# Nuttoty/Structured_Light_for_3D_Model_Replication

Hardware: AMD Instinct MI355X
Metric: decoded+triangulated px/s (higher is better)
Workload: dtype u8+f64

## Files before the change

### structured_light_for_3d_model_replication_amd/csrc/slgpu.hip

```cpp
#include <hip/hip_runtime.h>

#include <math.h>
#include <stdint.h>
#include <stdlib.h>
#include <string.h>

#include <stdio.h>

#include <algorithm>
#include <cmath>
#include <initializer_list>
#include <string>
#include <type_traits>
#include <thread>
#include <vector>

#include <dlfcn.h>
#include <errno.h>
#include <fcntl.h>
#include <sys/stat.h>
#include <unistd.h>

#include <chrono>
#include <condition_variable>
// ... 72 lines not shown
  int nc, nr, kc, kr;
  int mode;
  int Wp;
  const double4* planes;
  const float4* planes32;
  const double* xn;
  const double* yn;
  const float* xn32;
  const float* yn32;
  float fast_thr;
  int xy_safe;
  int xy_calc;
  double cx, cy, fx, fy;
  double rfx, rfy;
  const double* nc_rays;
  double o0, o1, o2;
  const double* poses;
  uint16_t* codes;
  int rec12;
  int rec_blk;
  uint8_t* ptnib;
  int32_t* col_out;
  int32_t* row_out;
  uint8_t* mask_out;
  void* xyz;
  uint8_t* bgr;
  int64_t out_cap;
  int64_t* view_offsets;
  ViewStats* stats;
  unsigned long long* masked;
  unsigned* hist;
  const int64_t* base_in;
  int* chunk_counts;
  int* block_sums;
  int bs_atomic;
  int decode_dyn;
  unsigned* super_base;
  unsigned* super_par;
  int sb_shift;
  int rerun;
  int cloud_gx;
  const uint8_t* pre_stack;
  int64_t pre_vs;
  unsigned* pre_hist;
  int pre_views;
  int pre_bpv;
};


__device__ __forceinline__ int64_t rec_slot(const Params& p, int view, int civ) {
  return (static_cast<int64_t>(civ >> 2) * p.n_views + view) * 4 + (civ & 3);
}

__device__ __forceinline__ uint4 ld16(const uint8_t* p, int n, bool vec) {
  if (vec) return *reinterpret_cast<const uint4*>(p);
  uint32_t w[4] = {0u, 0u, 0u, 0u};
#pragma unroll
  for (int i = 0; i < 16; ++i)
    if (i < n) w[i >> 2] |= static_cast<uint32_t>(p[i]) << (8 * (i & 3));
  return make_uint4(w[0], w[1], w[2], w[3]);
}

__device__ __forceinline__ uint32_t word(const uint4& q, int i) {
  return i == 0 ? q.x : i == 1 ? q.y : i == 2 ? q.z : q.w;
}

__device__ __forceinline__ uint32_t byte_of(const uint4& q, int i) {
  return (word(q, i >> 2) >> (8 * (i & 3))) & 0xffu;
}

__device__ __forceinline__ uint32_t gt_msb(uint32_t a, uint32_t b) {
  const uint32_t H = 0x80808080u;
  const uint32_t low = (a | H) - ((b & ~H) + 0x01010101u);
  return ((a & ~b) | (~(a ^ b) & low)) & H;
}

__device__ __forceinline__ uint32_t gt_bit7(uint32_t a, uint32_t b) {
  const uint32_t H = 0x80808080u;
  const uint32_t d = (b | H) - (a & ~H);
  return __builtin_amdgcn_bitop3_b32(a, b, d, 0x71);
}

__device__ __forceinline__ uint32_t gray_to_binary_bytes(uint32_t x, int bits) {
  if (bits > 1) x ^= (x >> 1) & 0x7f7f7f7fu;
// ... 255 lines not shown
}

template <int S>
__device__ __forceinline__ bool arrive_last(unsigned* ctr, unsigned id, unsigned readers) {
  const unsigned cls = id & (S - 1);
  const unsigned n_cls = (readers - cls + S - 1) / S;
  if (atomicAdd(ctr + 1 + cls, 1u) + 1u != n_cls) return false;
  return atomicAdd(ctr, 1u) + 1u == min(readers, static_cast<unsigned>(S));
}

__device__ __forceinline__ void hist_release(unsigned* h, int words, unsigned id, unsigned readers, int lane,
                                             uint32_t dep0, uint32_t dep1) {
  asm volatile("" ::"v"(dep0), "v"(dep1) : "memory");
  unsigned last = 0u;
  if (lane == 0) last = arrive_last<8>(h + kSlotArrive, id, readers) ? 1u : 0u;
  if (__shfl(static_cast<int>(last), 0, 64)) {
    uint4* h4 = reinterpret_cast<uint4*>(h);
    for (int i = lane; i < words / 4; i += 64) h4[i] = make_uint4(0u, 0u, 0u, 0u);
  }
}

__device__ __forceinline__ uint32_t mask4(uint32_t w, uint32_t b, uint32_t tw2, uint32_t tc2, uint32_t* bytes) {
  const uint32_t we = w & 0x00ff00ffu, wo = (w >> 8) & 0x00ff00ffu;
  const uint32_t be = b & 0x00ff00ffu, bo = (b >> 8) & 0x00ff00ffu;
  const uint32_t me = ((we | 0x80008000u) - tw2) & (((we + 0x00100010u) | 0x80008000u) - (be + tc2));
  const uint32_t mo = ((wo | 0x80008000u) - tw2) & (((wo + 0x00100010u) | 0x80008000u) - (bo + tc2));
  const uint32_t y = ((me >> 15) & 0x00010001u) | ((mo >> 7) & 0x01000100u);
  *bytes = y;
  return (y & 1u) | ((y >> 7) & 2u) | ((y >> 14) & 4u) | ((y >> 21) & 8u);
}

constexpr int kDecPl = 2048, kDecX = 4096, kDecY = 4096;
constexpr int kDecPlWords = kDecPl * 4;
constexpr int kBsSlots = 64;
constexpr int kSuperCap = 4096;
constexpr int kSuperWords = 2 * kSuperCap + 4;

__device__ __forceinline__ unsigned* super_produce(const Params& p) {
  const unsigned sel = p.super_par[0] & 1u;
  if (!p.rerun && blockIdx.x == 0 && blockIdx.y == 0) {
    unsigned* other = p.super_base + (sel ^ 1u) * kSuperCap;
    for (int i = threadIdx.x; i < kSuperCap; i += kThreads) other[i] = 0u;
    if (threadIdx.x == 0) p.super_par[1] = sel;
  }
  return p.super_base + sel * kSuperCap;
}
__device__ __forceinline__ const unsigned* super_consume(const Params& p, int bx) {
  const unsigned sel = p.super_par[1] & 1u;
  if (!p.rerun && bx == 0 && blockIdx.y == 0 && threadIdx.x == 0) p.super_par[0] = sel ^ 1u;
  return p.super_base + sel * kSuperCap;
}
constexpr int kDecodeLds = (kDecPlWords + kDecX) * 4;
static_assert(kDecodeLds >= 256 * kHistStride * 4, "the decode LDS holds the histogram replicas too");

constexpr int kDecodePerCu = 3;
template <int KC, int KR, int MODE, int VEC>
__global__ __launch_bounds__(kThreads, 3) void k_decode(Params p) {
  const int mode = MODE >= 0 ? MODE : p.mode;
  const int kc = KC >= 0 ? KC : p.kc;
  const int krr = (mode & M_ROWS) ? (KR >= 0 ? KR : p.kr) : 0;
  const int nc = p.nc, nr = p.nr;
  const bool vec = VEC > 0;
  const bool hist = (mode & M_HIST) && !(mode & M_DECIDE);

  __shared__ __attribute__((aligned(16))) unsigned s_lds[kDecodeLds / 4];
  __shared__ int s_max[kWaves];
  __shared__ int s_cnt[2][kWaves];
  __shared__ unsigned s_bsum[kBsSlots];
  __shared__ uint32_t s_thr[2];
  __shared__ unsigned s_mcount;
  __shared__ int s_next[2];
  __shared__ uint4 s_mapst[(MODE < 0 || (MODE & M_MAPS)) ? 64 * kWaves : 1];
  unsigned* s_hist = s_lds;
  float4* s_pl = reinterpret_cast<float4*>(s_lds);
  float* s_xn = reinterpret_cast<float*>(s_lds) + kDecPlWords;
  const bool decide = (mode & M_DECIDE) != 0;
  const int tid = threadIdx.x;
  const int lane = tid & 63;
  const int wid = __builtin_amdgcn_readfirstlane(tid >> 6);
  const int view = blockIdx.y;
  const int64_t HW = p.HW;
  const int gx = static_cast<int>(gridDim.x);
  if (decide) {
    if (tid < kBsSlots) s_bsum[tid] = 0u;
    if (tid == 0) s_mcount = 0u;
    if ((mode & M_HIST) && wid == 0) {
      const Thresholds t = view_thresholds(p, view, lane);
      if (lane == 0) {
        s_thr[0] = static_cast<uint32_t>(t.white + 1) * 0x00010001u;
        s_thr[1] = static_cast<uint32_t>(t.contrast + 17) * 0x00010001u;
        if (blockIdx.x == 0) {
          p.stats[view].thr_white = t.white;
          p.stats[view].thr_contrast = t.contrast;
          p.stats[view].noise_floor = t.noise_floor;
          p.stats[view].dynamic_range = t.dynamic_range;
        }
      }
    }
    if (mode & M_CODES) {
      const int wp_t = min(p.Wp, kDecPl), w_t = min(p.W, kDecX);
      typedef __attribute__((address_space(3))) void* lds_ptr_t;
      for (int i = wid; i * 64 < wp_t; i += kWaves)
        __builtin_amdgcn_global_load_lds(p.planes32 + min(i * 64 + lane, wp_t - 1), (lds_ptr_t)(s_pl + i * 64), 16, 0, 0);
      for (int i = wid; i * 256 < w_t; i += kWaves)
        __builtin_amdgcn_global_load_lds(p.xn32 + min(i * 256 + 4 * lane, w_t - 4), (lds_ptr_t)(s_xn + i * 256), 16, 0, 0);
    }
  }
  uint32_t tw2 = static_cast<uint32_t>(40 + 1) * 0x00010001u;
  uint32_t tc2 = static_cast<uint32_t>(10 + 17) * 0x00010001u;
  int it = 0;

  if (hist) {
    for (int i = tid; i < 256 * kHistStride; i += kThreads) s_hist[i] = 0u;
    __syncthreads();
  }

  const int ngroups = (p.cpv + kWaves - 1) / kWaves;
  int mx_acc = -1024;
  const bool dyn = p.decode_dyn && decide && (mode & M_CODES) && !p.bs_atomic;
  unsigned* const sup = (decide && (mode & M_CODES)) ? super_produce(p) : nullptr;
  unsigned* const dyn_ctr = sup + (kSuperCap - 1 - view);
  for (int cg = blockIdx.x; cg < ngroups;) {
  unsigned dyn_next = 0u;
  if (dyn && tid == 0) dyn_next = atomicAdd(dyn_ctr, 1u);
  const int civ = cg * kWaves + wid;
  const bool live = civ < p.cpv;
  const int64_t px0 = static_cast<int64_t>(civ) * kChunk + lane * kPx;
  const int n_px = live ? static_cast<int>(min<int64_t>(max<int64_t>(HW - px0, 0), kPx)) : 0;
  const int64_t pxl = n_px > 0 ? px0 : 0;
  const int64_t o = view * HW + px0;

  const float ys_early = (decide && (mode & M_CODES) && n_px > 0) ? p.yn32[row_of(p, static_cast<int>(px0))] : 0.0f;
  uint32_t col[kPx];
  uint32_t pt_rec = 0xffffu;
  uint4 wq = make_uint4(0u, 0u, 0u, 0u), bq = wq;
  uint32_t rA[4] = {0, 0, 0, 0}, rB[4] = {0, 0, 0, 0};
  const int rBn = krr > 8 ? krr - 8 : 0;
  const int rSh = nr - krr;
  if (mode & M_FROMMAPS) {
    const int64_t ol = view * HW + pxl;
    if (vec) {
      const int4* cm = reinterpret_cast<const int4*>(p.in_col + ol);
#pragma unroll
      for (int i = 0; i < 4; ++i) {
        const int4 v = cm[i];
        col[4 * i] = static_cast<uint32_t>(max(v.x, 0));
        col[4 * i + 1] = static_cast<uint32_t>(max(v.y, 0));
        col[4 * i + 2] = static_cast<uint32_t>(max(v.z, 0));
        col[4 * i + 3] = static_cast<uint32_t>(max(v.w, 0));
      }
    } else {
#pragma unroll
      for (int k = 0; k < kPx; ++k) col[k] = k < n_px ? static_cast<uint32_t>(max(p.in_col[ol + k], 0)) : 0u;
    }
  } else {
    const uint8_t* vbase = p.stack + view * p.stack_vs;
    const int voff = static_cast<int>(pxl);
    const __amdgpu_buffer_rsrc_t rs_view =
        __builtin_amdgcn_make_buffer_rsrc(const_cast<uint8_t*>(vbase), 0, p.view_bytes, 0x00020000);
// ... 180 lines not shown
      }
      const float ys = ys_early;
      uint32_t todo = ok;
      if (!(mode & M_NC)) {
#pragma unroll
        for (int k = 0; k < kPx; ++k) {
          const float a = fabsf(__builtin_fmaf(pf[k].x, xs[k], __builtin_fmaf(pf[k].y, ys, pf[k].z)));
          if (a > p.fast_thr) pt |= 1u << k;
        }
        pt &= ok;
        todo &= ~pt;
      }
#pragma unroll
      for (int k = 0; k < kPx; ++k) {
        if (!((todo >> k) & 1u)) continue;
        const int c = static_cast<int>(min(col[k], static_cast<uint32_t>(p.Wp - 1)));
        const int64_t q = px0 + k;
        float x, y, z, inv;
        if (mode & M_NC) {
          x = static_cast<float>(p.nc_rays[q]);
          y = static_cast<float>(p.nc_rays[HW + q]);
          z = static_cast<float>(p.nc_rays[2 * HW + q]);
          inv = 1.0f;
        } else {
          x = xs[k];
          y = ys;
          z = 1.0f;
          inv = __frsqrt_rn(x * x + y * y + 1.0f);
        }
        if (has_point(p, mode, pf[k], c, x, y, z, inv, u0 + k, v, q)) pt |= 1u << k;
      }
    }
    if (mode & M_CODES) {
      const int64_t gci = static_cast<int64_t>(view) * p.cpv + civ;
      pt_rec = pt;
      const int cnt = wave_sum_dpp(__popc(pt));
      if (lane == 0) {
        if (live) p.chunk_counts[gci] = cnt;
        const unsigned mine = live ? static_cast<unsigned>(cnt) : 0u;
        if (p.bs_atomic) {
          const unsigned old = atomicAdd(&s_bsum[it], (1u << 16) | mine);
          if ((old >> 16) == kWaves - 1) {
            const int64_t blk = static_cast<int64_t>(view) * ngroups + cg;
            const unsigned t = (old & 0xffffu) + mine;
            p.block_sums[blk] = static_cast<int>(t);
            if (t) atomicAdd(sup + (blk >> p.sb_shift), t);
          }
        } else {
          s_cnt[it & 1][wid] = static_cast<int>(mine);
        }
      }
    }
  }
  if (hist) {
    unsigned* hrow = s_hist + (lane & (kHistRep - 1));
    int mx = -1024;
#pragma unroll
    for (int k = 0; k < kPx; ++k) {
      if (k < n_px) {
        const int bk = static_cast<int>(byte_of(bq, k));
        atomicAdd(hrow + bk * kHistStride, 1u);
        mx = max(mx, static_cast<int>(byte_of(wq, k)) - bk);
      }
    }
    mx_acc = max(mx_acc, mx);
  }

  if (mode & M_CODES) {
    uint32_t rec[kPx / 2];
#pragma unroll
    for (int i = 0; i < kPx / 2; ++i)
      rec[i] = min(col[2 * i], static_cast<uint32_t>(p.Wp - 1)) |
               (min(col[2 * i + 1], static_cast<uint32_t>(p.Wp - 1)) << 16);
    if (decide) {
      const bool blk = !(mode & M_MAPS);
      if (n_px == kPx) {
        uint32_t rw[6];
        uint32_t* ro = blk ? rw : reinterpret_cast<uint32_t*>(reinterpret_cast<uint8_t*>(p.codes) + 3 * o / 2);
#pragma unroll
        for (int h = 0; h < 2; ++h) {
          const uint32_t* r = rec + 4 * h;
          auto cd = [&](int k, uint32_t c) { return ((pt_rec >> (8 * h + k)) & 1u) ? c : 0xfffu; };
          const uint32_t c0 = cd(0, r[0] & 0xffffu), c1 = cd(1, r[0] >> 16), c2 = cd(2, r[1] & 0xffffu);
          const uint32_t c3 = cd(3, r[1] >> 16), c4 = cd(4, r[2] & 0xffffu), c5 = cd(5, r[2] >> 16);
          const uint32_t c6 = cd(6, r[3] & 0xffffu), c7 = cd(7, r[3] >> 16);
          ro[3 * h] = c0 | (c1 << 12) | (c2 << 24);
          ro[3 * h + 1] = (c2 >> 8) | (c3 << 4) | (c4 << 16) | (c5 << 28);
          ro[3 * h + 2] = (c5 >> 4) | (c6 << 8) | (c7 << 20);
        }
        if (blk) {
          const __amdgpu_buffer_rsrc_t rs = __builtin_amdgcn_make_buffer_rsrc(
              reinterpret_cast<uint8_t*>(p.codes) + kRecSlot * rec_slot(p, view, civ), 0, kRecSlot, 0x00020000);
          __builtin_amdgcn_raw_buffer_store_b128(v4u{rw[0], rw[1], rw[2], rw[3]}, rs, 16 * lane, 0, kRecAux);
          __builtin_amdgcn_raw_buffer_store_b64(v2u{rw[4], rw[5]}, rs, 1024 + 8 * lane, 0, kRecAux);
        }
      }
    } else if (vec) {
      if (n_px == kPx) {
        uint4* ro = reinterpret_cast<uint4*>(p.codes + o);
        ro[0] = make_uint4(rec[0], rec[1], rec[2], rec[3]);
        ro[1] = make_uint4(rec[4], rec[5], rec[6], rec[7]);
      }
    } else {
#pragma unroll
      for (int k = 0; k < kPx; ++k)
        if (k < n_px) p.codes[o + k] = static_cast<uint16_t>(rec[k >> 1] >> (16 * (k & 1)));
    }
  }
  if (decide && (mode & M_CODES) && !p.bs_atomic) {
    if (dyn && tid == 0) s_next[it & 1] = static_cast<int>(dyn_next) + gx;
    __syncthreads();
    if (tid == 0) {
      int t = 0;
#pragma unroll
      for (int w = 0; w < kWaves; ++w) t += s_cnt[it & 1][w];
      const int64_t blk = static_cast<int64_t>(view) * ngroups + cg;
      p.block_sums[blk] = t;
      if (t) atomicAdd(sup + (blk >> p.sb_shift), static_cast<unsigned>(t));
    }
  }
  cg = dyn ? s_next[it & 1] : cg + gx;
  ++it;
  }

  if (decide && p.masked) {
    __syncthreads();
    if (tid == 0 && s_mcount) atomicAdd(p.masked + view, static_cast<unsigned long long>(s_mcount));
  }
  if (decide && (mode & M_HIST) && !p.rerun && wid == 0)
    hist_release(p.hist + static_cast<int64_t>(view) * kHistView, kHistView, blockIdx.x, gx, lane, tw2, tc2);

  if (hist) {
#pragma unroll
    for (int d = 32; d > 0; d >>= 1) mx_acc = max(mx_acc, __shfl_xor(mx_acc, d, 64));
    if (lane == 0) s_max[wid] = mx_acc;
    __syncthreads();
    unsigned* gh = p.hist + view * kSlot;
    unsigned cnt = 0u;
    const unsigned* row = s_hist + tid * kHistStride;
#pragma unroll
    for (int r = 0; r < kHistRep; ++r) cnt += row[r];
    if (cnt) atomicAdd(gh + tid, cnt);
    if (tid == 0) {
      int m = s_max[0];
#pragma unroll
      for (int w = 1; w < kWaves; ++w) m = max(m, s_max[w]);
      if (m > -1024) atomicMax(gh + 256, static_cast<unsigned>(m + 1024));
    }
  }
}

template <int VEC>
__device__ __forceinline__ int count_chunk(const Params& p, int64_t gc, int view, int civ, int lane, bool live,
                                           int* masked) {
// ... 185 lines not shown
          u -= W;
          ++v;
        }
        const int64_t q = static_cast<int64_t>(cpx) + 256 * s + 4 * lane + e;
        float x, y, z, inv;
        if (nc) {
          x = static_cast<float>(p.nc_rays[q]);
          y = static_cast<float>(p.nc_rays[p.HW + q]);
          z = static_cast<float>(p.nc_rays[2 * p.HW + q]);
          inv = 1.0f;
        } else {
          x = xs[e];
          y = vec ? ys : p.yn32[v];
          z = 1.0f;
          inv = __frsqrt_rn(x * x + y * y + 1.0f);
        }
        if (has_point(p, mode, pf[e], c, x, y, z, inv, u, v, q)) nib |= 1u << e;
      }
    }
    total += __popc(nib);
    nibs[s] = nib;
  }
#pragma unroll
  for (int s = 0; s < 4; ++s) p.ptnib[gc * kChunkNib + 64 * s + lane] = static_cast<uint8_t>(nibs[s]);
  if ((mode & M_MAPS) && vec) {
    uint8_t* mo_ = p.mask_out + static_cast<int64_t>(view) * HW;
#pragma unroll
    for (int s = 0; s < 4; ++s) {
      const int px = cpx + 256 * s + 4 * lane;
      if (px < HW) __builtin_nontemporal_store(mbytes[s], reinterpret_cast<uint32_t*>(mo_ + px));
    }
  }
  total = wave_sum(total);
  if (lane == 0) p.chunk_counts[gc] = total;
  return total;
}

template <int VEC>
__global__ __launch_bounds__(kThreads, 1) void k_count(Params p) {
  __shared__ int s_sum[kWaves];
  __shared__ int s_msum[kWaves];
  const int lane = threadIdx.x & 63;
  const int wid = __builtin_amdgcn_readfirstlane(threadIdx.x >> 6);
  const int view = blockIdx.y;
  const int civ = blockIdx.x * kWaves + wid;
  const int64_t gc = static_cast<int64_t>(view) * p.cpv + civ;
  int mc = 0;
  const int total = count_chunk<VEC>(p, gc, view, civ, lane, civ < p.cpv, &mc);
  if (p.masked) {
    mc = wave_sum(mc);
    if (lane == 0) s_msum[wid] = mc;
    __syncthreads();
    if (threadIdx.x == 0) {
      int t = 0;
#pragma unroll
      for (int w = 0; w < kWaves; ++w) t += s_msum[w];
      if (t) atomicAdd(p.masked + view, static_cast<unsigned long long>(t));
    }
  }
  if (!(p.mode & M_CODES)) return;
  unsigned* const sup = super_produce(p);
  if (lane == 0) s_sum[wid] = total;
  __syncthreads();
  if (threadIdx.x == 0) {
    int t = 0;
#pragma unroll
    for (int w = 0; w < kWaves; ++w) t += s_sum[w];
    const int64_t blk = static_cast<int64_t>(view) * gridDim.x + blockIdx.x;
    p.block_sums[blk] = t;
    if (t) atomicAdd(sup + (blk >> p.sb_shift), static_cast<unsigned>(t));
  }
}

constexpr int kPipe = 4;
constexpr int kBgrWords = 3 * kChunk / 4 + 4;

template <typename T>
__device__ __forceinline__ T* at_bytes(T* base, unsigned off) {
  using B = typename std::conditional<std::is_const<T>::value, const char, char>::type;
  return reinterpret_cast<T*>(reinterpret_cast<B*>(base) + off);
}

__device__ __forceinline__ uint32_t ent_code(uint32_t e) { return (e >> 10) & 0x7fffu; }
template <int VEC>
__device__ __forceinline__ void chunk_uv(int u_c, int v_c, uint32_t e, int W, int* u, int* v) {
  const int local = static_cast<int>(e & 1023u);
  int uu = u_c + local, vv = v_c;
  if (VEC > 0) {
    const int dr = static_cast<int>(e >> 25);
    uu -= dr * W;
    vv += dr;
  } else if (W >= kChunk) {
    const bool wrap = uu >= W;
    uu -= wrap ? W : 0;
    vv += wrap ? 1 : 0;
  } else {
    while (uu >= W) {
      uu -= W;
      ++vv;
    }
  }
  __builtin_assume(uu >= 0 && uu < (1 << 24));
// ... 423 lines not shown
      t4[3 * lane] = tq[0];
      t4[3 * lane + 1] = tq[1];
      t4[3 * lane + 2] = tq[2];
    } else {
      t4[lane] = tq[0];
    }
  }
  {
    int idx = incl - n_l;
#pragma unroll
    for (int k = 0; k < kPx; ++k) {
      const uint32_t code = (d[k >> 1] >> (16 * (k & 1))) & 0x7fffu;
      if ((ptbits >> k) & 1u) s_ent[idx] = static_cast<uint32_t>(lane * kPx + k) | (code << 10) | drow;
      idx += (ptbits >> k) & 1u;
    }
  }
  __builtin_amdgcn_wave_barrier();
  cloud_points<MODE, VEC, PIPE>(p, view, cpx, base, lane, total, s_ent, s_bgr);
}

constexpr int kPrefixBatch = 4;

__device__ __forceinline__ long long block_offset(const Params& p, const unsigned* sup, int64_t b, int tid, int lane,
                                                  int wid, long long* s_wred) {
  long long acc = 0;
  const int64_t sb = b >> p.sb_shift;
  for (int64_t t0 = 0; t0 < sb; t0 += kPrefixBatch * kThreads) {
    unsigned v[kPrefixBatch];
#pragma unroll
    for (int i = 0; i < kPrefixBatch; ++i) v[i] = sup[min<int64_t>(t0 + i * kThreads + tid, sb - 1)];
#pragma unroll
    for (int i = 0; i < kPrefixBatch; ++i) acc += (t0 + i * kThreads + tid < sb) ? v[i] : 0u;
  }
  for (int64_t t0 = sb << p.sb_shift; t0 < b; t0 += kPrefixBatch * kThreads) {
    int v[kPrefixBatch];
#pragma unroll
    for (int i = 0; i < kPrefixBatch; ++i) v[i] = p.block_sums[min<int64_t>(t0 + i * kThreads + tid, b - 1)];
#pragma unroll
    for (int i = 0; i < kPrefixBatch; ++i) acc += (t0 + i * kThreads + tid < b) ? v[i] : 0;
  }
  acc = wave_sum64(acc);
  if (lane == 0) s_wred[wid] = acc;
  __syncthreads();
  long long t = 0;
#pragma unroll
  for (int w = 0; w < kWaves; ++w) t += s_wred[w];
  return t;
}

constexpr int kExactPipe = 2;
constexpr int kVerifyPipe = 2;
static_assert(kWaves * kChunk >= 256 * kHistStride,
              "k_cloud's pre-stats workgroups keep their LDS histogram replicas in s_ent");
template <int MODE, int VEC, int PIPE>
__global__ __launch_bounds__(kThreads, 5) void k_cloud(Params p) {
  __shared__ uint32_t s_ent[kWaves][kChunk];
  __shared__ __attribute__((aligned(16))) uint32_t s_bgr[kWaves][kBgrWords];
  __shared__ long long s_wred[kWaves];
  const int tid = threadIdx.x;
  const int lane = tid & 63;
  const int wid = __builtin_amdgcn_readfirstlane(tid >> 6);
  const int view = blockIdx.y;
  const int npre = static_cast<int>(gridDim.x) - p.cloud_gx;
  if (static_cast<int>(blockIdx.x) < npre) {
    pre_stats_block(p, blockIdx.x, npre, &s_ent[0][0], reinterpret_cast<int*>(s_wred));
    return;
  }
  const int cx = static_cast<int>(blockIdx.x) - npre;
  const int civ = cx * kWaves + wid;
  const int64_t b = static_cast<int64_t>(view) * p.cloud_gx + cx;
  const int64_t gc = static_cast<int64_t>(view) * p.cpv + civ;
  const int before = (lane < wid && civ < p.cpv) ? p.chunk_counts[gc - wid + lane] : 0;
  long long base = block_offset(p, super_consume(p, cx), b, tid, lane, wid, s_wred);
  base += p.base_in ? *p.base_in : 0ll;
  base += wave_sum(before);
  base = uniform64(base);
  if (civ >= p.cpv) return;
  ChunkIn in;
  cloud_load<VEC>(p, gc, lane, &in);
  if (lane == 0 && view == p.n_views - 1 && civ == p.cpv - 1)
    p.view_offsets[p.n_views] = base + p.chunk_counts[gc];
  cloud_chunk<MODE, VEC, PIPE>(p, gc, base, lane, in, &s_ent[wid][0], &s_bgr[wid][0]);
}

}


struct sl_ctx {
  int device = 0;
  std::string err;
  bool has_calib = false;
  int H = 0, W = 0, Wp = 0;
  double Oc[3] = {0, 0, 0};
  double* d_planes = nullptr;
  double* d_xn = nullptr;
  double* d_yn = nullptr;
  float* d_f32 = nullptr;
  float fast_thr = 0.0f;
  bool xy_safe = false;
  bool xy_calc = false;
  bool xy_plain = false;
  bool planes_plain = false;
  double cam[4] = {0, 0, 1, 1};
  bool verify32 = true;
  double* d_nc = nullptr;
  ViewStats* d_stats = nullptr;
  int64_t cap_stats = 0;
  unsigned* d_hist[2] = {nullptr, nullptr};
  int64_t cap_hist = 0;
  int64_t hist_dirty[2] = {0, 0};
  unsigned long long cap_domain = 0;
  int* d_chunk_counts = nullptr;
  int64_t cap_cc = 0;
  int* d_block_sums = nullptr;
  int64_t cap_bs = 0;
  unsigned* d_super = nullptr;
  bool super_dirty = false;
  uint8_t* d_ptnib = nullptr;
  int64_t cap_ptnib = 0;
  uint16_t* d_codes = nullptr;
  int64_t cap_codes = 0;
  int last_views = 0;
  int decode_wgs = 0;
  int pre_wgs = 0;
  std::vector<hipEvent_t> prof_ev;
  std::vector<int> prof_groups;
  std::vector<char> prof_decide;
  int n_cu = 0;
  int prof_n = 0;
  void* comm = nullptr;
  int nranks = 0, rank = 0;
  int64_t* d_gcounts = nullptr;
  unsigned* d_ply_bsum = nullptr;
  int64_t cap_ply_bsum = 0;
  int64_t* d_ply_boff = nullptr;
  int64_t cap_ply_boff = 0;
  char* d_ply_text = nullptr;
  int64_t cap_ply_text = 0;
  char* h_ply_text = nullptr;
  int64_t cap_h_ply_text = 0;
  unsigned* d_plyr_state = nullptr;
  int64_t cap_plyr_state = 0;
  int64_t* d_plyr_tok = nullptr;
  int64_t cap_plyr_tok = 0;
  double* d_plyr_val = nullptr;
  int64_t cap_plyr_val = 0;
  int* d_plyr_cols = nullptr;
  int64_t cap_plyr_cols = 0;
// ... 89 lines not shown
      return fail((ctx), SL_EHIP, std::string(#expr) + ": " + hipGetErrorString(e_)); \
  } while (0)

int bit_count(int n) {
  int b = 0;
  while ((1ll << b) < n) ++b;
  return b;
}

int zero_async(sl_ctx* c, void* p, int64_t words, hipStream_t s);

template <typename T>
int grow(sl_ctx* c, T** ptr, int64_t* cap, int64_t need, hipStream_t s = nullptr, bool on_stream = false) {
  if (need <= *cap) return SL_OK;
  if (*ptr) HIP_TRY(c, hipFree(*ptr));
  *ptr = nullptr;
  const int64_t n = std::max<int64_t>(need, *cap * 2);
  const int64_t words = (static_cast<int64_t>(sizeof(T)) * n + 3) / 4;
  HIP_TRY(c, hipMalloc(reinterpret_cast<void**>(ptr), 4 * words));
  if (on_stream) {
    const int r = zero_async(c, *ptr, words, s);
    if (r) return r;
  } else {
    HIP_TRY(c, hipMemset(*ptr, 0, 4 * words));
    HIP_TRY(c, hipDeviceSynchronize());
  }
  *cap = n;
  return SL_OK;
}

int ensure_scratch(sl_ctx* c, int64_t views, int64_t px, bool codes, int64_t hist_views = 0,
                   bool* hist_fresh = nullptr, hipStream_t s = nullptr, bool on_stream = false) {
  const int64_t chunks = views * ((px + kChunk - 1) / kChunk);
  int r = grow(c, &c->d_chunk_counts, &c->cap_cc, chunks, s, on_stream);
  if (r) return r;
  r = grow(c, &c->d_block_sums, &c->cap_bs, views * (((px + kChunk - 1) / kChunk + kWaves - 1) / kWaves), s,
           on_stream);
  if (r) return r;
  r = grow(c, &c->d_ptnib, &c->cap_ptnib, chunks * kChunkNib, s, on_stream);
  if (r) return r;
  int64_t scap = c->d_super ? kSuperWords : 0;
  r = grow(c, &c->d_super, &scap, kSuperWords, s, on_stream);
  if (r) return r;
  const int64_t before = c->cap_hist, need = std::max(views, hist_views) * kHistView;
  for (int d = 0; d < 2; ++d) {
    int64_t cap = before;
    r = grow(c, &c->d_hist[d], &cap, need, s, on_stream);
    if (r) return r;
    if (d == 1) c->cap_hist = cap;
  }
  if (c->cap_hist != before) {
    c->hist_dirty[0] = c->hist_dirty[1] = 0;
    c->pre_armed = false;
    if (hist_fresh) *hist_fresh = true;
  }
  if (codes)
    return grow(c, &c->d_codes, &c->cap_codes,
                std::max<int64_t>(views * px, views * ((px + 4 * kChunk - 1) / (4 * kChunk)) * 4 * (kRecSlot / 2)) + 16,
                s, on_stream);
  return SL_OK;
}

using KernelFn = void (*)(Params);
constexpr int kProfGroups = 64;
constexpr int kProfEv = 4 * kProfGroups;

KernelFn pick_decode(int kc, int kr, int mode, bool vec) {
  if (vec && !(mode & (M_NC | M_FROMMAPS))) {
    constexpr int mrch = M_MAPS | M_ROWS | M_CODES | M_HIST, mrh = M_MAPS | M_ROWS | M_HIST,
                  ch = M_CODES | M_HIST, mrc = M_MAPS | M_ROWS | M_CODES, cc = M_CODES;
// ... 115 lines not shown
    pc.pre_views = pnv;
    pc.pre_bpv = static_cast<int>(bpv);
    const int64_t total = static_cast<int64_t>(pnv) * bpv;
    grid.x += static_cast<unsigned>((total + nv - 1) / nv);
    hist_dirty = static_cast<int64_t>(pnv) * kHistView;
  };
  bool next_pre = pre_use;
  int g = 0;
  for (int v0 = 0; v0 < p0.n_views; v0 += vpg, ++g) {
    hipEvent_t* gev = (ev && g < kProfGroups) ? ev + 4 * g : nullptr;
    if (gev) HIP_TRY(c, hipEventRecord(gev[0], s));
    const int nv = std::min(vpg, p0.n_views - v0);
    c->last_launch_px = static_cast<int64_t>(nv) * p0.HW;
    Params p = p0;
    p.n_views = nv;
    p.n_chunks = static_cast<int64_t>(nv) * cpv;
    if (p.stack) p.stack += v0 * p.stack_vs;
    if (p.tex) p.tex += v0 * p.tex_vs;
    if (p.in_col) p.in_col += v0 * p.HW;
    if (p.in_mask) p.in_mask += v0 * p.HW;
    if (p.col_out) p.col_out += v0 * p.HW;
    if (p.row_out) p.row_out += v0 * p.HW;
    if (p.mask_out) p.mask_out += v0 * p.HW;
    if (p.poses) p.poses += 16 * v0;
    if (p.masked) p.masked += v0;
    if (p.view_offsets) p.view_offsets += v0;
    p.base_in = (v0 > 0 && p.view_offsets) ? p.view_offsets : nullptr;
    p.stats = c->d_stats + v0;
    p.codes = c->d_codes;
    p.rec12 = (decide && cloud_mode >= 0) ? 1 : 0;
    p.rec_blk = (p.rec12 && !(decode_mode & M_MAPS)) ? 1 : 0;
    p.ptnib = c->d_ptnib;
    p.chunk_counts = c->d_chunk_counts;
    p.block_sums = c->d_block_sums;
    p.hist = hbuf;
    p.super_base = c->d_super;
    p.super_par = c->d_super + 2 * kSuperCap;
    const bool pre_g = next_pre;
    next_pre = false;
    const dim3 grid(static_cast<unsigned>((cpv + kWaves - 1) / kWaves), static_cast<unsigned>(nv));
    {
      const int64_t nb = static_cast<int64_t>(grid.x) * nv;
      int sh = 0;
      while ((int64_t{1} << (2 * sh)) < nb) ++sh;
      p.sb_shift = sh;
    }
    c->last.valid = true;
    dim3 dgrid = grid;
    if (c->decode_wgs > 0) dgrid.x = std::min(grid.x, static_cast<unsigned>(std::max(1, (c->decode_wgs + nv - 1) / nv)));
    c->last.grid[0] = dgrid;
    p.bs_atomic = decide && (grid.x + dgrid.x - 1) / dgrid.x <= static_cast<unsigned>(kBsSlots);
    p.decode_dyn = (!(decode_mode & M_MAPS) && decide && codes && dgrid.x < grid.x &&
                    ((static_cast<int64_t>(grid.x) * nv) >> p.sb_shift) + 1 + nv < kSuperCap) ? 1 : 0;
    if (p.decode_dyn) p.bs_atomic = 0;
    c->last.grid[1] = c->last.grid[2] = grid;
    c->last.s = s;
    c->last.fn[1] = c->last.fn[2] = nullptr;
    c->last.decide = decide;
    c->last.stats = false;
    if (decide) {
      if (adaptive) {
        const int64_t per_view = (p0.HW / 16 + kThreads - 1) / kThreads;
        const dim3 sg(static_cast<unsigned>(std::max<int64_t>(1, std::min<int64_t>(per_view, (2 * c->n_cu + nv - 1) / nv))),
                      static_cast<unsigned>(nv));
        p.mode = decode_mode;
        c->last.p[1] = p;
        c->last.grid[1] = sg;
        c->last.stats = true;
        if (!pre_g) {
          void* args[] = {&p};
          const void* kst = reinterpret_cast<const void*>(k_stats);
          c->last.fn[1] = kst;
          HIP_TRY(c, hipLaunchKernel(kst, sg, dim3(kThreads), args, 0, s));
        }
      }
      if (gev) HIP_TRY(c, hipEventRecord(gev[1], s));
    }
    if (codes) c->super_dirty = true;
    {
      p.mode = decode_mode;
      KernelFn fn = pick_decode(p.kc, (decode_mode & M_ROWS) ? p.kr : 0, decode_mode, vec);
      c->last.p[0] = p;
      c->last.p[0].masked = nullptr;
      c->last.fn[0] = reinterpret_cast<const void*>(fn);
      void* args[] = {&p};
      HIP_TRY(c, hipLaunchKernel(reinterpret_cast<const void*>(fn), dgrid, dim3(kThreads), args, 0, s));
      hist_dirty = (adaptive && !decide) ? static_cast<int64_t>(nv) * kSlot : 0;
// ... 442 lines not shown
    n_cu = 256;
  c->n_cu = n_cu;
  c->decode_wgs = kDecodePerCu * n_cu;
  c->pre_wgs = 2 * n_cu;
  if (const char* d = getenv("SLGPU_VERIFY32")) c->verify32 = atoi(d) != 0;
  if (hipEventCreateWithFlags(&c->done_ev, hipEventDisableTiming) != hipSuccess) {
    delete c;
    return SL_EHIP;
  }
  *out = c;
  return SL_OK;
}

void sl_ctx_destroy(sl_ctx* c) {
  if (!c) return;
  (void)hipSetDevice(c->device);
  if (c->comm) {
    if (Rccl* R = rccl()) (void)R->comm_destroy(static_cast<ncclComm_t>(c->comm));
  }
  if (c->d_gcounts) (void)hipFree(c->d_gcounts);
  for (void* ptr : {static_cast<void*>(c->d_ply_bsum), static_cast<void*>(c->d_ply_boff),
                    static_cast<void*>(c->d_ply_text), static_cast<void*>(c->d_plyr_state),
                    static_cast<void*>(c->d_plyr_tok), static_cast<void*>(c->d_plyr_val),
                    static_cast<void*>(c->d_plyr_cols)})
    if (ptr) (void)hipFree(ptr);
  if (c->h_ply_text) (void)hipHostFree(c->h_ply_text);
  slstream::ring_release(&c->file_ring);
  if (c->done_ev) (void)hipEventDestroy(c->done_ev);
  for (hipEvent_t e : c->prof_ev) (void)hipEventDestroy(e);
  for (void* ptr : {static_cast<void*>(c->d_planes), static_cast<void*>(c->d_xn), static_cast<void*>(c->d_yn),
                    static_cast<void*>(c->d_nc), static_cast<void*>(c->d_stats), static_cast<void*>(c->d_f32),
                    static_cast<void*>(c->d_codes), static_cast<void*>(c->d_hist[0]),
                    static_cast<void*>(c->d_hist[1]), static_cast<void*>(c->d_ptnib),
                    static_cast<void*>(c->d_block_sums), static_cast<void*>(c->d_chunk_counts),
                    static_cast<void*>(c->d_super)})
    if (ptr) (void)hipFree(ptr);
  delete c;
}

const char* sl_ctx_last_error(const sl_ctx* c) { return c ? c->err.c_str() : "null context"; }

int sl_ctx_reserve(sl_ctx* c, int64_t max_views, int64_t max_px) {
  if (!c || max_views < 1 || max_px < 1) return fail(c, SL_EINVAL, "sl_ctx_reserve: bad sizes");
  HIP_TRY(c, hipSetDevice(c->device));
  const int64_t vpg = std::max<int64_t>(1, kMaxChunks / ((max_px + kChunk - 1) / kChunk));
  int r = ensure_scratch(c, std::min(vpg, max_views), max_px, true, vpg);
  if (r) return r;
  return grow(c, &c->d_stats, &c->cap_stats, max_views);
}

int sl_set_calib(sl_ctx* c, int H, int W, const double* K, const double* Oc, const double* planes,
                 int Wp, const double* Nc) {
  if (!c) return SL_EINVAL;
  if (H < 1 || W < 1 || Wp < 1 || !K || !Oc || !planes)
    return fail(c, SL_EINVAL, "sl_set_calib: bad arguments");
  if (Wp > kMaxWp) return fail(c, SL_EINVAL, "sl_set_calib: at most 32768 projector columns");
  HIP_TRY(c, hipSetDevice(c->device));
  const double fx = K[0], fy = K[4], cx = K[2], cy = K[5];
  std::vector<double> xn(W), yn(H);
  for (int u = 0; u < W; ++u) xn[u] = (static_cast<double>(u) - cx) / fx;
  for (int v = 0; v < H; ++v) yn[v] = (static_cast<double>(v) - cy) / fy;
  bool use_nc = false;
  const int64_t HW = static_cast<int64_t>(H) * W;
  if (Nc) {
    for (int64_t q = 0; q < HW && !use_nc; ++q) {
      const double x = xn[q % W], y = yn[q / W];
      const double nrm = sqrt((x * x + y * y) + 1.0);
// ... 413 lines not shown
  hipError_t e = clear();
  if (e == hipSuccess && c->last.decide && c->last.stats) e = run(reinterpret_cast<const void*>(k_stats), 1);
  if (e == hipSuccess) e = run(c->last.fn[0], 0);
  if (e == hipSuccess && !c->last.decide && c->last.fn[1]) e = run(c->last.fn[1], 1);
  hipEvent_t ev[4] = {nullptr, nullptr, nullptr, nullptr};
  for (int k = 0; k < 4 && e == hipSuccess; ++k) e = hipEventCreate(&ev[k]);
  int r = e == hipSuccess ? SL_OK : fail(c, SL_EHIP, std::string("sl_time_kernels: ") + hipGetErrorString(e));
  const int order3[3] = {2, 1, 0}, orderd[3] = {2, 0, 1};
  const int* order = c->last.decide ? orderd : order3;
  if (r == SL_OK && hipEventRecord(ev[0], s) != hipSuccess) r = fail(c, SL_EHIP, "hipEventRecord");
  for (int q = 0; q < 3 && r == SL_OK; ++q) {
    const int k = order[q];
    if (c->last.fn[k]) {
      for (int i = 0; i < reps; ++i) {
        e = run(c->last.fn[k], k);
        if (e != hipSuccess) {
          r = fail(c, SL_EHIP, std::string("sl_time_kernels: ") + hipGetErrorString(e));
          break;
        }
      }
    }
    if (r == SL_OK && hipEventRecord(ev[q + 1], s) != hipSuccess) r = fail(c, SL_EHIP, "hipEventRecord");
  }
  double out[3] = {0.0, 0.0, 0.0};
  if (r == SL_OK && hipEventSynchronize(ev[3]) == hipSuccess) {
    for (int q = 0; q < 3; ++q) {
      float ms = 0.f;
      const int k = order[q];
      if (hipEventElapsedTime(&ms, ev[q], ev[q + 1]) == hipSuccess) out[k] = c->last.fn[k] ? ms / reps : 0.0;
    }
  }
  if (r == SL_OK && c->last.fn[0] && c->last.p[0].decode_dyn) {
    const unsigned nv = c->last.grid[0].y;
    unsigned* ctr = c->d_super + (kSuperCap - nv);
    double sum = 0.0;
    for (int i = 0; i < reps && r == SL_OK; ++i) {
      float ms = 0.f;
      if (hipMemsetAsync(ctr, 0, sizeof(unsigned) * nv, s) != hipSuccess || hipEventRecord(ev[0], s) != hipSuccess ||
          run(c->last.fn[0], 0) != hipSuccess || hipEventRecord(ev[1], s) != hipSuccess ||
          hipEventSynchronize(ev[1]) != hipSuccess || hipEventElapsedTime(&ms, ev[0], ev[1]) != hipSuccess) {
        r = fail(c, SL_EHIP, "sl_time_kernels: dynamic k_decode re-run");
        break;
      }
      sum += ms;
    }
    if (r == SL_OK) out[0] = sum / reps;
  }
  for (int k = 0; k < 4; ++k)
    if (ev[k]) (void)hipEventDestroy(ev[k]);
  if (clear() != hipSuccess && r == SL_OK) r = fail(c, SL_EHIP, "sl_time_kernels: scratch reset");
  c->hist_dirty[0] = c->hist_dirty[1] = 0;
  c->super_dirty = r != SL_OK;
  c->pre_armed = false;
  c->last.valid = false;
  if (decode_ms) *decode_ms = out[0];
  if (count_ms) *count_ms = out[1];
  if (cloud_ms) *cloud_ms = out[2];
  return r;
}

int sl_last_launch_info(sl_ctx* c, int* path, int64_t* launches, int64_t* last_launch_px) {
  if (!c) return SL_EINVAL;
  if (path) *path = c->last.decide ? 1 : 0;
  if (launches) *launches = c->last_launches;
  if (last_launch_px) *last_launch_px = c->last_launch_px;
  return SL_OK;
}

int sl_last_thresholds(sl_ctx* c, int view, float* nf, float* dr, int* thr_w, int* thr_c) {
  if (!c) return SL_EINVAL;
  if (view < 0 || view >= c->last_views || !c->d_stats) return fail(c, SL_EINVAL, "no such view");
// ... 291 lines not shown
```

Before: 78.88 billion.

## Drop block_sums; schedule decode chunks per wave with padded per-view atomic counters

Removes the block_sums buffer and the per-iteration __syncthreads reduction in k_decode. Each wave now claims its own chunk from a dynamic counter, and the counters for different views are spaced apart by a stride to avoid contention on shared cache lines. Lane 0 of each wave adds its chunk count straight into the super-block sums. Chunk counts are padded to a multiple of kWaves so the prefix pass can read them as int4 in place of block sums. This trades block barriers for more global atomics per wave and larger padded count storage.

```diff
diff --git a/structured_light_for_3d_model_replication_amd/csrc/slgpu.hip b/structured_light_for_3d_model_replication_amd/csrc/slgpu.hip
--- a/structured_light_for_3d_model_replication_amd/csrc/slgpu.hip
+++ b/structured_light_for_3d_model_replication_amd/csrc/slgpu.hip
@@ -128,9 +128,8 @@
   unsigned* hist;
   const int64_t* base_in;
   int* chunk_counts;
-  int* block_sums;
-  int bs_atomic;
   int decode_dyn;
+  int ctr_stride;
   unsigned* super_base;
   unsigned* super_par;
   int sb_shift;
@@ -146,6 +145,10 @@
 
 __device__ __forceinline__ int64_t rec_slot(const Params& p, int view, int civ) {
   return (static_cast<int64_t>(civ >> 2) * p.n_views + view) * 4 + (civ & 3);
+}
+
+__device__ __forceinline__ int64_t cc_slot(const Params& p, int view, int civ) {
+  return static_cast<int64_t>(view) * ((p.cpv + kWaves - 1) / kWaves * kWaves) + civ;
 }
 
 __device__ __forceinline__ uint4 ld16(const uint8_t* p, int n, bool vec) {
@@ -467,7 +470,6 @@
 
 constexpr int kDecPl = 2048, kDecX = 4096, kDecY = 4096;
 constexpr int kDecPlWords = kDecPl * 4;
-constexpr int kBsSlots = 64;
 constexpr int kSuperCap = 4096;
 constexpr int kSuperWords = 2 * kSuperCap + 4;
 
@@ -500,11 +502,8 @@
 
   __shared__ __attribute__((aligned(16))) unsigned s_lds[kDecodeLds / 4];
   __shared__ int s_max[kWaves];
-  __shared__ int s_cnt[2][kWaves];
-  __shared__ unsigned s_bsum[kBsSlots];
   __shared__ uint32_t s_thr[2];
   __shared__ unsigned s_mcount;
-  __shared__ int s_next[2];
   __shared__ uint4 s_mapst[(MODE < 0 || (MODE & M_MAPS)) ? 64 * kWaves : 1];
   unsigned* s_hist = s_lds;
   float4* s_pl = reinterpret_cast<float4*>(s_lds);
@@ -517,7 +516,6 @@
   const int64_t HW = p.HW;
   const int gx = static_cast<int>(gridDim.x);
   if (decide) {
-    if (tid < kBsSlots) s_bsum[tid] = 0u;
     if (tid == 0) s_mcount = 0u;
     if ((mode & M_HIST) && wid == 0) {
       const Thresholds t = view_thresholds(p, view, lane);
@@ -552,14 +550,18 @@
 
   const int ngroups = (p.cpv + kWaves - 1) / kWaves;
   int mx_acc = -1024;
-  const bool dyn = p.decode_dyn && decide && (mode & M_CODES) && !p.bs_atomic;
+  const bool dyn = p.decode_dyn && decide && (mode & M_CODES);
   unsigned* const sup = (decide && (mode & M_CODES)) ? super_produce(p) : nullptr;
-  unsigned* const dyn_ctr = sup + (kSuperCap - 1 - view);
-  for (int cg = blockIdx.x; cg < ngroups;) {
+  unsigned* const dyn_ctr = sup + (kSuperCap - 1 - view * p.ctr_stride);
+  for (int civ = blockIdx.x * kWaves + wid; it == 0 || civ < p.cpv;) {
+  const bool live = civ < p.cpv;
   unsigned dyn_next = 0u;
-  if (dyn && tid == 0) dyn_next = atomicAdd(dyn_ctr, 1u);
-  const int civ = cg * kWaves + wid;
-  const bool live = civ < p.cpv;
+  if (dyn && live && lane == 0) {
+    typedef __attribute__((address_space(1))) unsigned* global_ptr_t;
+    global_ptr_t ctr = (global_ptr_t)dyn_ctr;
+    asm volatile("" : "+v"(ctr));
+    dyn_next = __hip_atomic_fetch_add(ctr, 1u, __ATOMIC_RELAXED, __HIP_MEMORY_SCOPE_AGENT);
+  }
   const int64_t px0 = static_cast<int64_t>(civ) * kChunk + lane * kPx;
   const int n_px = live ? static_cast<int>(min<int64_t>(max<int64_t>(HW - px0, 0), kPx)) : 0;
   const int64_t pxl = n_px > 0 ? px0 : 0;
@@ -806,22 +808,16 @@
       }
     }
     if (mode & M_CODES) {
-      const int64_t gci = static_cast<int64_t>(view) * p.cpv + civ;
       pt_rec = pt;
       const int cnt = wave_sum_dpp(__popc(pt));
-      if (lane == 0) {
-        if (live) p.chunk_counts[gci] = cnt;
-        const unsigned mine = live ? static_cast<unsigned>(cnt) : 0u;
-        if (p.bs_atomic) {
-          const unsigned old = atomicAdd(&s_bsum[it], (1u << 16) | mine);
-          if ((old >> 16) == kWaves - 1) {
-            const int64_t blk = static_cast<int64_t>(view) * ngroups + cg;
-            const unsigned t = (old & 0xffffu) + mine;
-            p.block_sums[blk] = static_cast<int>(t);
-            if (t) atomicAdd(sup + (blk >> p.sb_shift), t);
-          }
-        } else {
-          s_cnt[it & 1][wid] = static_cast<int>(mine);
+      if (live) {
+        int* const cc = p.chunk_counts + cc_slot(p, view, civ);
+        if (lane == 0) {
+          *cc = cnt;
+          const int64_t blk = static_cast<int64_t>(view) * ngroups + civ / kWaves;
+          if (cnt) atomicAdd(sup + (blk >> p.sb_shift), static_cast<unsigned>(cnt));
+        } else if (civ == p.cpv - 1 && civ + lane < ngroups * kWaves) {
+          cc[lane] = 0;
         }
       }
     }
@@ -881,19 +877,10 @@
         if (k < n_px) p.codes[o + k] = static_cast<uint16_t>(rec[k >> 1] >> (16 * (k & 1)));
     }
   }
-  if (decide && (mode & M_CODES) && !p.bs_atomic) {
-    if (dyn && tid == 0) s_next[it & 1] = static_cast<int>(dyn_next) + gx;
-    __syncthreads();
-    if (tid == 0) {
-      int t = 0;
-#pragma unroll
-      for (int w = 0; w < kWaves; ++w) t += s_cnt[it & 1][w];
-      const int64_t blk = static_cast<int64_t>(view) * ngroups + cg;
-      p.block_sums[blk] = t;
-      if (t) atomicAdd(sup + (blk >> p.sb_shift), static_cast<unsigned>(t));
-    }
-  }
-  cg = dyn ? s_next[it & 1] : cg + gx;
+  if (dyn)
+    civ = live ? gx * kWaves + static_cast<int>(__builtin_amdgcn_readfirstlane(dyn_next)) : p.cpv;
+  else
+    civ += gx * kWaves;
   ++it;
   }
 
@@ -1145,7 +1132,7 @@
     }
   }
   total = wave_sum(total);
-  if (lane == 0) p.chunk_counts[gc] = total;
+  if (lane == 0) p.chunk_counts[cc_slot(p, view, civ)] = total;
   return total;
 }
 
@@ -1160,6 +1147,7 @@
   const int64_t gc = static_cast<int64_t>(view) * p.cpv + civ;
   int mc = 0;
   const int total = count_chunk<VEC>(p, gc, view, civ, lane, civ < p.cpv, &mc);
+  if (civ >= p.cpv && lane == 0) p.chunk_counts[cc_slot(p, view, civ)] = 0;
   if (p.masked) {
     mc = wave_sum(mc);
     if (lane == 0) s_msum[wid] = mc;
@@ -1180,7 +1168,6 @@
 #pragma unroll
     for (int w = 0; w < kWaves; ++w) t += s_sum[w];
     const int64_t blk = static_cast<int64_t>(view) * gridDim.x + blockIdx.x;
-    p.block_sums[blk] = t;
     if (t) atomicAdd(sup + (blk >> p.sb_shift), static_cast<unsigned>(t));
   }
 }
@@ -1670,12 +1657,13 @@
 #pragma unroll
     for (int i = 0; i < kPrefixBatch; ++i) acc += (t0 + i * kThreads + tid < sb) ? v[i] : 0u;
   }
+  const int4* const cc4 = reinterpret_cast<const int4*>(p.chunk_counts);
   for (int64_t t0 = sb << p.sb_shift; t0 < b; t0 += kPrefixBatch * kThreads) {
-    int v[kPrefixBatch];
-#pragma unroll
-    for (int i = 0; i < kPrefixBatch; ++i) v[i] = p.block_sums[min<int64_t>(t0 + i * kThreads + tid, b - 1)];
-#pragma unroll
-    for (int i = 0; i < kPrefixBatch; ++i) acc += (t0 + i * kThreads + tid < b) ? v[i] : 0;
+    int4 v[kPrefixBatch];
+#pragma unroll
+    for (int i = 0; i < kPrefixBatch; ++i) v[i] = cc4[min<int64_t>(t0 + i * kThreads + tid, b - 1)];
+#pragma unroll
+    for (int i = 0; i < kPrefixBatch; ++i) acc += (t0 + i * kThreads + tid < b) ? v[i].x + v[i].y + v[i].z + v[i].w : 0;
   }
   acc = wave_sum64(acc);
   if (lane == 0) s_wred[wid] = acc;
@@ -1708,7 +1696,8 @@
   const int civ = cx * kWaves + wid;
   const int64_t b = static_cast<int64_t>(view) * p.cloud_gx + cx;
   const int64_t gc = static_cast<int64_t>(view) * p.cpv + civ;
-  const int before = (lane < wid && civ < p.cpv) ? p.chunk_counts[gc - wid + lane] : 0;
+  const int64_t cc = cc_slot(p, view, civ);
+  const int before = (lane < wid && civ < p.cpv) ? p.chunk_counts[cc - wid + lane] : 0;
   long long base = block_offset(p, super_consume(p, cx), b, tid, lane, wid, s_wred);
   base += p.base_in ? *p.base_in : 0ll;
   base += wave_sum(before);
@@ -1717,7 +1706,7 @@
   ChunkIn in;
   cloud_load<VEC>(p, gc, lane, &in);
   if (lane == 0 && view == p.n_views - 1 && civ == p.cpv - 1)
-    p.view_offsets[p.n_views] = base + p.chunk_counts[gc];
+    p.view_offsets[p.n_views] = base + p.chunk_counts[cc];
   cloud_chunk<MODE, VEC, PIPE>(p, gc, base, lane, in, &s_ent[wid][0], &s_bgr[wid][0]);
 }
 
@@ -1750,8 +1739,6 @@
   unsigned long long cap_domain = 0;
   int* d_chunk_counts = nullptr;
   int64_t cap_cc = 0;
-  int* d_block_sums = nullptr;
-  int64_t cap_bs = 0;
   unsigned* d_super = nullptr;
   bool super_dirty = false;
   uint8_t* d_ptnib = nullptr;
@@ -1907,10 +1894,8 @@
 int ensure_scratch(sl_ctx* c, int64_t views, int64_t px, bool codes, int64_t hist_views = 0,
                    bool* hist_fresh = nullptr, hipStream_t s = nullptr, bool on_stream = false) {
   const int64_t chunks = views * ((px + kChunk - 1) / kChunk);
-  int r = grow(c, &c->d_chunk_counts, &c->cap_cc, chunks, s, on_stream);
-  if (r) return r;
-  r = grow(c, &c->d_block_sums, &c->cap_bs, views * (((px + kChunk - 1) / kChunk + kWaves - 1) / kWaves), s,
-           on_stream);
+  int r = grow(c, &c->d_chunk_counts, &c->cap_cc,
+               views * (((px + kChunk - 1) / kChunk + kWaves - 1) / kWaves * kWaves), s, on_stream);
   if (r) return r;
   r = grow(c, &c->d_ptnib, &c->cap_ptnib, chunks * kChunkNib, s, on_stream);
   if (r) return r;
@@ -2092,7 +2077,6 @@
     p.rec_blk = (p.rec12 && !(decode_mode & M_MAPS)) ? 1 : 0;
     p.ptnib = c->d_ptnib;
     p.chunk_counts = c->d_chunk_counts;
-    p.block_sums = c->d_block_sums;
     p.hist = hbuf;
     p.super_base = c->d_super;
     p.super_par = c->d_super + 2 * kSuperCap;
@@ -2109,10 +2093,10 @@
     dim3 dgrid = grid;
     if (c->decode_wgs > 0) dgrid.x = std::min(grid.x, static_cast<unsigned>(std::max(1, (c->decode_wgs + nv - 1) / nv)));
     c->last.grid[0] = dgrid;
-    p.bs_atomic = decide && (grid.x + dgrid.x - 1) / dgrid.x <= static_cast<unsigned>(kBsSlots);
-    p.decode_dyn = (!(decode_mode & M_MAPS) && decide && codes && dgrid.x < grid.x &&
-                    ((static_cast<int64_t>(grid.x) * nv) >> p.sb_shift) + 1 + nv < kSuperCap) ? 1 : 0;
-    if (p.decode_dyn) p.bs_atomic = 0;
+    const int64_t n_sums = ((static_cast<int64_t>(grid.x) * nv) >> p.sb_shift) + 1;
+    p.decode_dyn = (!(decode_mode & M_MAPS) && decide && codes && dgrid.x < grid.x && n_sums + nv < kSuperCap) ? 1 : 0;
+    p.ctr_stride = static_cast<int>(std::max<int64_t>(1, (kSuperCap - n_sums) / nv));
+    if (p.ctr_stride >= 32) p.ctr_stride &= ~31;
     c->last.grid[1] = c->last.grid[2] = grid;
     c->last.s = s;
     c->last.fn[1] = c->last.fn[2] = nullptr;
@@ -2621,7 +2605,7 @@
                     static_cast<void*>(c->d_nc), static_cast<void*>(c->d_stats), static_cast<void*>(c->d_f32),
                     static_cast<void*>(c->d_codes), static_cast<void*>(c->d_hist[0]),
                     static_cast<void*>(c->d_hist[1]), static_cast<void*>(c->d_ptnib),
-                    static_cast<void*>(c->d_block_sums), static_cast<void*>(c->d_chunk_counts),
+                    static_cast<void*>(c->d_chunk_counts),
                     static_cast<void*>(c->d_super)})
     if (ptr) (void)hipFree(ptr);
   delete c;
@@ -3101,11 +3085,12 @@
   }
   if (r == SL_OK && c->last.fn[0] && c->last.p[0].decode_dyn) {
     const unsigned nv = c->last.grid[0].y;
-    unsigned* ctr = c->d_super + (kSuperCap - nv);
+    const size_t span = static_cast<size_t>(nv - 1) * c->last.p[0].ctr_stride + 1;
+    unsigned* ctr = c->d_super + (kSuperCap - span);
     double sum = 0.0;
     for (int i = 0; i < reps && r == SL_OK; ++i) {
       float ms = 0.f;
-      if (hipMemsetAsync(ctr, 0, sizeof(unsigned) * nv, s) != hipSuccess || hipEventRecord(ev[0], s) != hipSuccess ||
+      if (hipMemsetAsync(ctr, 0, sizeof(unsigned) * span, s) != hipSuccess || hipEventRecord(ev[0], s) != hipSuccess ||
           run(c->last.fn[0], 0) != hipSuccess || hipEventRecord(ev[1], s) != hipSuccess ||
           hipEventSynchronize(ev[1]) != hipSuccess || hipEventElapsedTime(&ms, ev[0], ev[1]) != hipSuccess) {
         r = fail(c, SL_EHIP, "sl_time_kernels: dynamic k_decode re-run");
```

Result: slower. 72.28 billion (-8.4%).
